# ZrrSkywalker/MonoDETR

Measured on NVIDIA H100. Metric: images/sec (1280x384, fwd+bwd), higher is better.
Workload: dtype f32 (BF16x3: error-compensated bf16 tensor-core products, fp32 accumulate)

## Files before the change

monodetr_b200/csrc/conv_gemm.cu:

```cuda
#include <cuda.h>
#include <cuda_runtime.h>
#include <stdint.h>
#include <stdlib.h>
#include <string.h>

#include "../../include/monodetr_b200.h"
#include "launch.cuh"
#include "tc_common.cuh"
#include "tma_host.cuh"

namespace {

using namespace mdb;

constexpr int BM = 128;
constexpr int BK = 32;
constexpr int kTileABytes = BM * 128;
constexpr int kChunkBytes = 32 * 128;
constexpr int kConsumerThreads = 256;
constexpr int kThreadsTC = kConsumerThreads + 32;
constexpr int kMaxTaps = 9;

struct TcParams {
    int tiles_x, tiles_y, tw, th, tb;
    int Ho, Wo;
    int out_sy, out_sx, out_oy, out_ox, out_H, out_W;
    int in_sy, in_sx;
    int ntaps, cblocks;
    int tap_dy[kMaxTaps], tap_dx[kMaxTaps], tap_w[kMaxTaps];
    int rtiles_x, rtiles_y, rtw, rth, n_img, red_per_split;
    int kb_per_slice, slice_stride;
    int total_tiles, n_tiles_n, n_tiles_m;
    int w_sy, w_sx, wg_taps, wg_kw, wg_pad;
    int Mo_rows;
    int No, ldo;
    int relu, atomic_out, round_out;
    int epi_tma, epi_load, half_x, half_y, half_b;
    const float* bias;
    const float* residual;
    const float* relu_mask;
    const float* rowscale;
    float* out;
};

template <bool MN>
__device__ __forceinline__ uint32_t raw_off(int row, int k) {
    if constexpr (MN) return (uint32_t)((row >> 5) * kChunkBytes + k * 128 + (((((row & 31) >> 2) ^ (k & 7))) << 4) + (row & 3) * 4);
    else return (uint32_t)(row * 128 + (((k >> 2) ^ (row & 7)) << 4) + (k & 3) * 4);
}

__device__ __forceinline__ float trunc_tf32(float x) { return __uint_as_float(__float_as_uint(x) & 0xFFFFE000u); }

template <int BN, int STAGES, int MODE, int PREC>
struct TcSmem {
    static constexpr bool kConvB = !(PREC == 2 && MODE == 0);
    static constexpr int kRing = STAGES * (kTileABytes + BN * 128);
    static constexpr int kStage = 2 * 64 * BN * 4;
    static constexpr int kConv = kConvB ? (PREC == 1 ? 2 : 1) * BN * 128 : 0;
    static constexpr int kFixed = kRing + kConv + 1024  + 256 ;
    static constexpr bool kTmaEpi = MODE == 0 && kFixed + kStage <= 227 * 1024;
    static constexpr int kBytes = kFixed + (kTmaEpi ? kStage : 0);
};

template <int BN, int STAGES, int MODE , bool B_MN, int PREC>
__global__ void __launch_bounds__(kThreadsTC, 1)
tc_conv_gemm_kernel(const __grid_constant__ CUtensorMap mapA, const __grid_constant__ CUtensorMap mapB,
                    const __grid_constant__ CUtensorMap mapO, const __grid_constant__ CUtensorMap mapR,
                    const __grid_constant__ TcParams p) {
    constexpr bool A_MN = (MODE == 1);
    static_assert(!(MODE == 1) || B_MN, "wgrad reads both operands MN-major");
    static_assert(BN == 64 || BN == 128, "tile width");
    constexpr bool BF_B = (PREC == 2 && MODE == 0);
    static_assert(!BF_B || !B_MN, "pre-split weights are K-major");
    constexpr bool CONVB = !BF_B;
    constexpr int kTileBBytes = BN * 128;
    constexpr int kRawBytes = kTileABytes + kTileBBytes;
    using SM = TcSmem<BN, STAGES, MODE, PREC>;
    constexpr int NACC = BN / 2;

    extern __shared__ __align__(1024) uint8_t smem[];
    uint8_t* stage_out = smem + STAGES * kRawBytes;
    uint8_t* bconv = stage_out + (SM::kTmaEpi ? SM::kStage : 0);
    uint64_t* full_bar = reinterpret_cast<uint64_t*>(bconv + SM::kConv);
    uint64_t* empty_bar = full_bar + STAGES;
    uint64_t* epi_bar = empty_bar + STAGES;

    const int warp = threadIdx.x >> 5;
    const int lane = threadIdx.x & 31;

    struct Tile { int n0, img, y0, x0, m0, red_begin, iters, tap, slice; };
    auto decode = [&](int tix) {
        Tile t;
        t.n0 = (tix % p.n_tiles_n) * BN;
        int r = tix / p.n_tiles_n;
        t.img = t.y0 = t.x0 = t.m0 = t.red_begin = t.tap = t.slice = 0;
        if constexpr (MODE == 0) {
            const int per_img = p.tiles_x * p.tiles_y;
            t.iters = p.ntaps * p.cblocks;
            if (p.kb_per_slice > 0) {
                t.slice = r / p.n_tiles_m;
                r -= t.slice * p.n_tiles_m;
                t.red_begin = t.slice * p.kb_per_slice;
                t.iters = max(0, min(t.iters, t.red_begin + p.kb_per_slice) - t.red_begin);
            }
            const int grp = r / per_img;
            t.img = grp * p.tb;
            r -= grp * per_img;
            t.y0 = (r / p.tiles_x) * p.th;
            t.x0 = (r % p.tiles_x) * p.tw;
        } else {
            t.m0 = (r % p.n_tiles_m) * BM;
// ... 34 lines not shown
                const Tile t = decode(tix);
                for (int it = 0; it < t.iters; ++it, ++git) {
                    const int s = git % STAGES;
                    const uint32_t ph = (git / STAGES) & 1;
                    mbar_wait(&empty_bar[s], ph ^ 1);
                    uint8_t* a_dst = smem + s * kRawBytes;
                    uint8_t* b_dst = a_dst + kTileABytes;
                    mbar_arrive_expect_tx(&full_bar[s], kRawBytes);
                    if constexpr (MODE == 0) {
                        const int kit = t.red_begin + it;
                        const int tap = kit / p.cblocks;
                        const int cb = kit - tap * p.cblocks;
                        tma_load_4d(a_dst, &mapA, &full_bar[s], cb * BK, t.x0 * p.in_sx + p.tap_dx[tap],
                                    t.y0 * p.in_sy + p.tap_dy[tap], t.img);
                        if constexpr (BF_B) {
                            tma_load_3d(b_dst, &mapB, &full_bar[s], cb * 64, t.n0, p.tap_w[tap]);
                        } else if constexpr (!B_MN) {
                            tma_load_3d(b_dst, &mapB, &full_bar[s], cb * BK, t.n0, p.tap_w[tap]);
                        } else {
#pragma unroll
                            for (int j = 0; j < BN / 32; ++j)
                                tma_load_3d(b_dst + j * kChunkBytes, &mapB, &full_bar[s], t.n0 + j * 32, cb * BK, p.tap_w[tap]);
                        }
                    } else {
                        int r = t.red_begin + it;
                        const int per_img = p.rtiles_x * p.rtiles_y;
                        const int ri = r / per_img;
                        r -= ri * per_img;
                        const int ry = (r / p.rtiles_x) * p.rth;
                        const int rx = (r % p.rtiles_x) * p.rtw;
#pragma unroll
                        for (int j = 0; j < BM / 32; ++j)
                            tma_load_4d(a_dst + j * kChunkBytes, &mapA, &full_bar[s], t.m0 + j * 32, rx, ry, ri);
#pragma unroll
                        for (int j = 0; j < BN / 32; ++j)
                            tma_load_4d(b_dst + j * kChunkBytes, &mapB, &full_bar[s], t.n0 + j * 32,
                                        rx * p.w_sx + (t.tap % p.wg_kw) - p.wg_pad, ry * p.w_sy + (t.tap / p.wg_kw) - p.wg_pad, ri);
                    }
                }
            }
        }
        return;
    }
    if (warp > kConsumerThreads / 32) return;

    const int wg = warp >> 2;
    const int g = lane >> 2, tig = lane & 3;
    const int r0 = wg * 64 + (warp & 3) * 16 + g;
    const int ctid = threadIdx.x;
    const bool epi_tma = SM::kTmaEpi && p.epi_tma;
    const bool leader = (ctid & 127) == 0;
    uint8_t* my_stage = stage_out + wg * (SM::kStage / 2);
    uint32_t epi_phase = 0;
    int git = 0;
    for (int tix = blockIdx.x; tix < p.total_tiles; tix += gridDim.x) {
        const Tile t = decode(tix);
        if (p.atomic_out && t.iters == 0) continue;
        const int c1 = t.x0 + wg * p.half_x, c2 = t.y0 + wg * p.half_y, c3 = t.img + wg * p.half_b, c4 = t.slice;
        if (epi_tma && p.epi_load && leader) {
            bulk_wait_read_all();
            mbar_arrive_expect_tx(&epi_bar[wg], SM::kStage / 2);
#pragma unroll
            for (int c = 0; c < BN / 32; ++c) tma_load_5d(my_stage + c * 8192, &mapR, &epi_bar[wg], t.n0 + 32 * c, c1, c2, c3, c4);
        }
        float acc[NACC];
#pragma unroll
        for (int i = 0; i < NACC; ++i) acc[i] = 0.f;
        for (int it = 0; it < t.iters; ++it, ++git) {
            const int s = git % STAGES;
            const uint32_t ph = (git / STAGES) & 1;
            mbar_wait(&full_bar[s], ph);
            const uint8_t* a_raw = smem + s * kRawBytes;
            const uint8_t* b_raw = a_raw + kTileABytes;
            if constexpr (CONVB) {
                named_bar_sync(1, kConsumerThreads);
                if constexpr (PREC == 2) {
#pragma unroll
                    for (int i = ctid; i < BN * 4; i += kConsumerThreads) {
                        const int n = i % BN, c = i / BN;
                        float x[8];
#pragma unroll
                        for (int e = 0; e < 8; ++e) x[e] = *reinterpret_cast<const float*>(b_raw + raw_off<B_MN>(n, 8 * c + e));
                        uint32_t hw[4], lw[4];
#pragma unroll
                        for (int e = 0; e < 4; ++e) {
                            const uint32_t h = pack_bf16x2(x[2 * e], x[2 * e + 1]);
                            hw[e] = h;
                            lw[e] = pack_bf16x2(x[2 * e] - __uint_as_float(h << 16), x[2 * e + 1] - __uint_as_float(h & 0xFFFF0000u));
                        }
                        uint8_t* brow = bconv + n * 128;
                        *reinterpret_cast<uint4*>(brow + ((c ^ (n & 7)) << 4)) = make_uint4(hw[0], hw[1], hw[2], hw[3]);
                        *reinterpret_cast<uint4*>(brow + (((4 + c) ^ (n & 7)) << 4)) = make_uint4(lw[0], lw[1], lw[2], lw[3]);
                    }
                } else {
#pragma unroll 4
                    for (int i = ctid; i < BN * 8; i += kConsumerThreads) {
                        const int n = i % BN, c = i / BN;
                        float4 x;
                        if constexpr (B_MN) {
                            x.x = *reinterpret_cast<const float*>(b_raw + raw_off<true>(n, 4 * c));
                            x.y = *reinterpret_cast<const float*>(b_raw + raw_off<true>(n, 4 * c + 1));
                            x.z = *reinterpret_cast<const float*>(b_raw + raw_off<true>(n, 4 * c + 2));
                            x.w = *reinterpret_cast<const float*>(b_raw + raw_off<true>(n, 4 * c + 3));
                        } else {
                            x = *reinterpret_cast<const float4*>(b_raw + raw_off<false>(n, 4 * c));
                        }
                        const float4 h = make_float4(trunc_tf32(x.x), trunc_tf32(x.y), trunc_tf32(x.z), trunc_tf32(x.w));
                        const uint32_t off = n * 128 + ((c ^ (n & 7)) << 4);
                        *reinterpret_cast<float4*>(bconv + off) = h;
                        if constexpr (PREC == 1)
                            *reinterpret_cast<float4*>(bconv + kTileBBytes + off) = make_float4(x.x - h.x, x.y - h.y, x.z - h.z, x.w - h.w);
                    }
                }
                fence_proxy_async_smem();
                named_bar_sync(1, kConsumerThreads);
            }
            const uint32_t b_addr = smem_u32(CONVB ? bconv : b_raw);
            constexpr int KS = PREC == 2 ? 2 : 4;
            uint32_t ahi[KS][4], alo[KS][4];
#pragma unroll
            for (int ks = 0; ks < KS; ++ks) {
#pragma unroll
                for (int f = 0; f < 4; ++f) {
                    const int row = r0 + (f & 1) * 8;
                    if constexpr (PREC == 2) {
                        const int k = ks * 16 + tig * 2 + (f >> 1) * 8;
                        float x0, x1;
                        if constexpr (A_MN) {
                            x0 = *reinterpret_cast<const float*>(a_raw + raw_off<true>(row, k));
                            x1 = *reinterpret_cast<const float*>(a_raw + raw_off<true>(row, k + 1));
                        } else {
                            const float2 v = *reinterpret_cast<const float2*>(a_raw + raw_off<false>(row, k));
                            x0 = v.x; x1 = v.y;
                        }
                        const uint32_t h = pack_bf16x2(x0, x1);
                        ahi[ks][f] = h;
                        alo[ks][f] = pack_bf16x2(x0 - __uint_as_float(h << 16), x1 - __uint_as_float(h & 0xFFFF0000u));
                    } else {
                        const int k = ks * 8 + tig + (f >> 1) * 4;
                        const float x = *reinterpret_cast<const float*>(a_raw + raw_off<A_MN>(row, k));
                        const float h = trunc_tf32(x);
                        ahi[ks][f] = __float_as_uint(h);
                        alo[ks][f] = __float_as_uint(x - h);
                    }
                }
            }
            wgmma_fence();
#pragma unroll
            for (int ks = 0; ks < KS; ++ks) {
                const uint64_t bhi = make_wgmma_desc_sw128(b_addr + ks * 32);
                const uint64_t blo = make_wgmma_desc_sw128(b_addr + (PREC == 2 ? 64 : kTileBBytes) + ks * 32);
                if constexpr (PREC == 2) {
                    if constexpr (BN == 128) {
                        wgmma_bf16_n128(acc, ahi[ks], bhi, 1);
                        wgmma_bf16_n128(acc, alo[ks], bhi, 1);
                        wgmma_bf16_n128(acc, ahi[ks], blo, 1);
                    } else {
                        wgmma_bf16_n64(acc, ahi[ks], bhi, 1);
                        wgmma_bf16_n64(acc, alo[ks], bhi, 1);
                        wgmma_bf16_n64(acc, ahi[ks], blo, 1);
                    }
                } else {
                    if constexpr (BN == 128) wgmma_tf32_n128(acc, ahi[ks], bhi, 1);
                    else wgmma_tf32_n64(acc, ahi[ks], bhi, 1);
                    if constexpr (PREC == 1) {
                        if constexpr (BN == 128) {
                            wgmma_tf32_n128(acc, alo[ks], bhi, 1);
                            wgmma_tf32_n128(acc, ahi[ks], blo, 1);
                        } else {
                            wgmma_tf32_n64(acc, alo[ks], bhi, 1);
                            wgmma_tf32_n64(acc, ahi[ks], blo, 1);
                        }
                    }
                }
            }
            wgmma_commit();
            wgmma_wait_all();
            wgmma_fence_operands(acc);
            __syncwarp();
            if (lane == 0) mbar_arrive(&empty_bar[s]);
        }

        if (epi_tma) {
            if (p.epi_load) {
                mbar_wait(&epi_bar[wg], epi_phase);
                epi_phase ^= 1;
            } else {
                if (leader) bulk_wait_read_all();
                named_bar_sync(2 + wg, 128);
            }
#pragma unroll
            for (int h = 0; h < 2; ++h) {
                const int row = r0 + h * 8, rr = row - 64 * wg;
                const float* gmask = nullptr;
                if (p.relu_mask && p.epi_load != 2) {
                    const int lyt = row / p.tw, lx = row - lyt * p.tw;
                    const int ib = lyt / p.th, ly = lyt - ib * p.th;
                    const int y = t.y0 + ly, x = t.x0 + lx, img = t.img + ib;
                    if ((y < p.Ho) && (x < p.Wo) && (img < p.n_img))
                        gmask = p.relu_mask + (size_t)((img * p.out_H + y * p.out_sy + p.out_oy) * p.out_W + x * p.out_sx + p.out_ox) * p.ldo;
                }
#pragma unroll
                for (int j = 0; j < BN / 8; ++j) {
                    const int n = t.n0 + j * 8 + tig * 2;
                    if (n >= p.No) continue;
                    float2* sp = reinterpret_cast<float2*>(my_stage + (j >> 2) * 8192 + raw_off<false>(rr, (j & 3) * 8 + tig * 2));
                    float v[2] = {acc[4 * j + 2 * h], acc[4 * j + 2 * h + 1]};
                    if (p.bias) { v[0] += p.bias[n]; v[1] += p.bias[n + 1]; }
                    if (p.epi_load == 1) { const float2 e = *sp; v[0] += e.x; v[1] += e.y; }
                    if (p.relu) { v[0] = fmaxf(v[0], 0.f); v[1] = fmaxf(v[1], 0.f); }
                    if (p.relu_mask) {
                        float2 m = make_float2(0.f, 0.f);
                        if (p.epi_load == 2) m = *sp;
                        else if (gmask) m = *reinterpret_cast<const float2*>(gmask + n);
                        v[0] = m.x > 0.f ? v[0] : 0.f; v[1] = m.y > 0.f ? v[1] : 0.f;
                    }
                    if (p.round_out) { v[0] = round_tf32(v[0]); v[1] = round_tf32(v[1]); }
                    *sp = make_float2(v[0], v[1]);
                }
            }
            fence_proxy_async_smem();
            named_bar_sync(2 + wg, 128);
            if (leader) {
#pragma unroll
                for (int c = 0; c < BN / 32; ++c) tma_store_5d(&mapO, my_stage + c * 8192, t.n0 + 32 * c, c1, c2, c3, c4);
                bulk_commit();
            }
            continue;
        }
#pragma unroll
        for (int h = 0; h < 2; ++h) {
            const int row = r0 + h * 8;
            bool ok;
            size_t roff;
            float rsc = 1.f;
            if constexpr (MODE == 0) {
                const int lyt = row / p.tw, lx = row - lyt * p.tw;
                const int ib = lyt / p.th, ly = lyt - ib * p.th;
                const int y = t.y0 + ly, x = t.x0 + lx, img = t.img + ib;
                ok = (y < p.Ho) && (x < p.Wo) && (img < p.n_img);
                const int oy = y * p.out_sy + p.out_oy, ox = x * p.out_sx + p.out_ox;
                roff = (size_t)((img * p.out_H + oy) * p.out_W + ox) * p.ldo + (size_t)t.slice * p.slice_stride;
            } else {
                ok = (t.m0 + row) < p.Mo_rows;
                if (ok && p.rowscale) rsc = p.rowscale[t.m0 + row];
                roff = (size_t)(t.tap * p.Mo_rows + t.m0 + row) * p.ldo;
            }
            if (!ok) continue;
            const bool vec = !(p.ldo & 1);
#pragma unroll
            for (int j = 0; j < BN / 8; ++j) {
                const int n = t.n0 + j * 8 + tig * 2;
                if (n >= p.No) continue;
                float v[2] = {acc[4 * j + 2 * h] * rsc, acc[4 * j + 2 * h + 1] * rsc};
                const bool pair = vec && n + 1 < p.No;
                if (p.bias) { v[0] += p.bias[n]; if (pair) v[1] += p.bias[n + 1]; }
                if (p.residual) {
                    if (pair) { const float2 e = *reinterpret_cast<const float2*>(p.residual + roff + n); v[0] += e.x; v[1] += e.y; }
                    else v[0] += p.residual[roff + n];
                }
                if (p.relu) { v[0] = fmaxf(v[0], 0.f); v[1] = fmaxf(v[1], 0.f); }
                if (p.relu_mask) {
                    if (pair) {
                        const float2 m = *reinterpret_cast<const float2*>(p.relu_mask + roff + n);
                        v[0] = m.x > 0.f ? v[0] : 0.f; v[1] = m.y > 0.f ? v[1] : 0.f;
                    } else {
                        v[0] = p.relu_mask[roff + n] > 0.f ? v[0] : 0.f;
                    }
                }
                if (p.round_out) { v[0] = round_tf32(v[0]); v[1] = round_tf32(v[1]); }
                float* dst = p.out + roff + n;
// ... 91 lines not shown
void pick_tile(int W, int H, int n_pix, int* tw, int* th) {
    int best_tw = n_pix, best_waste = 1 << 30;
    for (int w = n_pix; w >= 1; w >>= 1) {
        const int h = n_pix / w;
        const int tx = (W + w - 1) / w, ty = (H + h - 1) / h;
        const int waste = tx * w * ty * h - W * H;
        if (waste < best_waste) { best_waste = waste; best_tw = w; }
    }
    *tw = best_tw;
    *th = n_pix / best_tw;
}

void pick_tile3(int W, int H, int B, int n_pix, int* tw, int* th, int* tb) {
    long long best = -1;
    *tw = n_pix; *th = 1; *tb = 1;
    for (int b = 1; b <= n_pix; b <<= 1)
        for (int w = n_pix / b; w >= 1; w >>= 1) {
            const int h = n_pix / b / w;
            if (b > 1 && b >= 2 * B) continue;
            const long long cov = (long long)((W + w - 1) / w) * w * ((H + h - 1) / h) * h * ((B + b - 1) / b) * b;
            if (best < 0 || cov < best) { best = cov; *tw = w; *th = h; *tb = b; }
        }
}

bool aligned16(const void* q) { return (reinterpret_cast<uintptr_t>(q) & 15u) == 0; }

int setup_epi_px(TcParams& p, CUtensorMap* mo, CUtensorMap* mr, size_t off, int Wc, int Hc, int B, uint64_t sx, uint64_t sy,
                 uint64_t sb, int slices) {
    p.epi_tma = p.epi_load = p.half_x = p.half_y = p.half_b = 0;
    if (p.No % 4 || p.ldo % 4 || !aligned16(p.out + off) || (p.residual && !aligned16(p.residual + off)) ||
        (p.relu_mask && !aligned16(p.relu_mask + off)))
        return 0;
    uint32_t box[5] = {32, (uint32_t)p.tw, (uint32_t)p.th, (uint32_t)p.tb, 1};
    if (p.tb > 1) p.half_b = box[3] = p.tb / 2;
    else if (p.th > 1) p.half_y = box[2] = p.th / 2;
    else p.half_x = box[1] = p.tw / 2;
    if (box[1] > 256 || box[2] > 256 || box[3] > 256) return 0;
    uint64_t dims[5] = {(uint64_t)p.No, (uint64_t)Wc, (uint64_t)Hc, (uint64_t)B, (uint64_t)slices};
    uint64_t str[5] = {1, sx, sy, sb, slices > 1 ? (uint64_t)p.slice_stride : sb * B};
    int rc = make_map(mo, p.out + off, 5, dims, str, box, nullptr);
    if (rc) return rc;
    const float* opnd = p.residual ? p.residual : p.relu_mask;
    if (opnd) {
        rc = make_map(mr, opnd + off, 5, dims, str, box, nullptr);
        if (rc) return rc;
        p.epi_load = p.residual ? 1 : 2;
    }
    p.epi_tma = 1;
    return 0;
}

int launch_fwd(const CUtensorMap& ma, const CUtensorMap& mb, const CUtensorMap& mo, const CUtensorMap& mr, const TcParams& p, dim3 grid, int bn, int precision, cudaStream_t stream) {
    if (precision == 2) return bn == 64 ? launch_tc<64, 6, 0, false, 2>(ma, mb, mo, mr, p, grid, stream) : launch_tc<128, 5, 0, false, 2>(ma, mb, mo, mr, p, grid, stream);
    if (precision == 1) return bn == 64 ? launch_tc<64, 5, 0, false, 1>(ma, mb, mo, mr, p, grid, stream) : launch_tc<128, 4, 0, false, 1>(ma, mb, mo, mr, p, grid, stream);
    return bn == 64 ? launch_tc<64, 6, 0, false, 0>(ma, mb, mo, mr, p, grid, stream) : launch_tc<128, 5, 0, false, 0>(ma, mb, mo, mr, p, grid, stream);
}

struct ConvGeom {
    int B, H, W, Cin, Cout, kh, kw, stride, pad, Ho, Wo;
};

int check_geom(const ConvGeom& g, bool forward = false) {
    if (g.B <= 0 || g.H <= 0 || g.W <= 0 || g.Cin <= 0 || g.Cout <= 0) return MDB_EINVAL;
    if (g.kh != g.kw || (g.kh != 1 && g.kh != 3) || (g.stride != 1 && g.stride != 2)) return MDB_EUNSUPPORTED;
    if (g.Cin % 4 || (!forward && g.Cout % 4)) return MDB_EUNSUPPORTED;
    return 0;
}

}

extern "C" {

int mdb_set_precision(int mode) {
    if (mode < 0 || mode > 2) return MDB_EINVAL;
    g_precision = mode;
    return 0;
}
int mdb_get_precision(void) { return g_precision; }

}

namespace {

int forward_splitk_slices(int precision, int kblocks, int bn, bool plain_epilogue, int Cout, long long out_elems) {
    const int kb_per_slice = 32;
    if (precision == 0 || bn != 128 || kblocks < 256 || !plain_epilogue || Cout % 4) return 0;
    const int slices = (kblocks + kb_per_slice - 1) / kb_per_slice;
    return (out_elems * slices < (1ll << 31)) ? slices : 0;
}

int conv_forward_impl(const float* x, const void* w_packed, bool bf, const float* bias, const float* residual, float* y,
                      int B, int H, int W, int Cin, int Cout, int kh, int kw, int stride, int pad, int flags,
                      void* stream_, size_t* query_ws = nullptr ) {
    const int precision = bf ? 2 : (g_precision == 2 ? 1 : g_precision);
    ConvGeom g{B, H, W, Cin, Cout, kh, kw, stride, pad, (H + 2 * pad - kh) / stride + 1, (W + 2 * pad - kw) / stride + 1};
    int rc = check_geom(g, true);
    if (rc) return rc;
    if (!query_ws && (!x || !w_packed || !y)) return MDB_EINVAL;
    if ((unsigned long long)B * g.Ho * g.Wo * Cout >= (1ull << 31)) return MDB_EUNSUPPORTED;
    cudaStream_t stream = static_cast<cudaStream_t>(stream_);
    if (kh == 1 && stride == 1 && pad == 0) {
        W = B * H * W; H = 1; B = 1;
        g = ConvGeom{B, H, W, Cin, Cout, kh, kw, stride, pad, H, W};
    }
    TcParams p;
    memset(&p, 0, sizeof(p));
    pick_tile3(g.Wo, g.Ho, B, BM, &p.tw, &p.th, &p.tb);
// ... 106 lines not shown
            p.Ho = Hc; p.Wo = Wc;
            p.out_sy = p.out_sx = stride; p.out_oy = py; p.out_ox = px; p.out_H = H; p.out_W = W;
            p.in_sy = p.in_sx = 1;
            p.cblocks = (Cout + BK - 1) / BK;
            int nt = 0;
            for (int ky = 0; ky < kh; ++ky) {
                if ((py + pad - ky) % stride) continue;
                for (int kx = 0; kx < kw; ++kx) {
                    if ((px + pad - kx) % stride) continue;
                    p.tap_dy[nt] = (py + pad - ky) / stride;
                    p.tap_dx[nt] = (px + pad - kx) / stride;
                    p.tap_w[nt] = ky * kw + kx;
                    ++nt;
                }
            }
            p.ntaps = nt;
            p.wg_taps = 1; p.wg_kw = 1;
            p.No = Cin; p.ldo = Cin; p.relu = 0; p.atomic_out = 0; p.round_out = (precision == 0) ? ((flags >> 1) & 1) : 0;
            p.bias = nullptr; p.residual = residual; p.relu_mask = relu_mask; p.rowscale = nullptr; p.out = dx;
            CUtensorMap ma, mb;
            {
                uint64_t dims[4] = {(uint64_t)Cout, (uint64_t)g.Wo, (uint64_t)g.Ho, (uint64_t)B};
                uint64_t str[4] = {1, (uint64_t)Cout, (uint64_t)g.Wo * Cout, (uint64_t)g.Ho * g.Wo * Cout};
                uint32_t box[4] = {BK, (uint32_t)p.tw, (uint32_t)p.th, (uint32_t)p.tb};
                rc = make_map(&ma, dy, 4, dims, str, box, nullptr);
                if (rc) return rc;
            }
            const int bn = (bf && Cin <= 64) ? 64 : 128;
            if (bf) {
                const uint64_t kb = (uint64_t)p.cblocks;
                uint64_t dims[3] = {64 * kb, (uint64_t)Cin, (uint64_t)(kh * kw)};
                uint64_t str[3] = {1, 64 * kb, (uint64_t)Cin * 64 * kb};
                uint32_t box[3] = {64, (uint32_t)bn, 1};
                rc = make_map(&mb, w_packed, 3, dims, str, box, nullptr, true);
                if (rc) return rc;
            } else {
                uint64_t dims[3] = {(uint64_t)Cin, (uint64_t)Cout, (uint64_t)(kh * kw)};
                uint64_t str[3] = {1, (uint64_t)Cin, (uint64_t)Cout * Cin};
                uint32_t box[3] = {32, 32, 1};
                rc = make_map(&mb, w_packed, 3, dims, str, box, nullptr);
                if (rc) return rc;
            }
            dim3 grid((Cin + bn - 1) / bn, n_groups * p.tiles_x * p.tiles_y, 1);
            if (nt == 0) {
                p.ntaps = 0;
            }
            CUtensorMap mo, mr;
            memset(&mo, 0, sizeof(mo));
            memset(&mr, 0, sizeof(mr));
            rc = setup_epi_px(p, &mo, &mr, (size_t)(py * W + px) * Cin, Wc, Hc, B, (uint64_t)stride * Cin,
                              (uint64_t)stride * W * Cin, (uint64_t)H * W * Cin, 1);
            if (rc) return rc;
            if (bf) rc = launch_fwd(ma, mb, mo, mr, p, grid, bn, 2, stream);
            else rc = (precision == 1) ? launch_tc<128, 4, 0, true, 1>(ma, mb, mo, mr, p, grid, stream)
                                       : launch_tc<128, 5, 0, true, 0>(ma, mb, mo, mr, p, grid, stream);
            if (rc) return rc;
        }
    return 0;
}

}

extern "C" {

int mdb_conv2d_forward_f32(const float* x, const float* w_packed, const float* bias, const float* residual, float* y,
                           int B, int H, int W, int Cin, int Cout, int kh, int kw, int stride, int pad, int flags,
                           void* stream) {
    return conv_forward_impl(x, w_packed, false, bias, residual, y, B, H, W, Cin, Cout, kh, kw, stride, pad, flags, stream);
}
int mdb_conv2d_forward_bf16x3(const float* x, const void* w_split, const float* bias, const float* residual, float* y,
                              int B, int H, int W, int Cin, int Cout, int kh, int kw, int stride, int pad, int flags,
                              void* stream) {
    return conv_forward_impl(x, w_split, true, bias, residual, y, B, H, W, Cin, Cout, kh, kw, stride, pad, flags, stream);
}
long long mdb_conv2d_forward_workspace_bytes(int B, int H, int W, int Cin, int Cout, int kh, int kw, int stride, int pad,
                                             int flags, int has_residual, int split_weights) {
    size_t bytes = 0;
    const float* res = has_residual ? reinterpret_cast<const float*>(16) : nullptr;
    const int rc = conv_forward_impl(nullptr, nullptr, split_weights != 0, nullptr, res, nullptr, B, H, W, Cin, Cout, kh, kw, stride,
                                     pad, flags, nullptr, &bytes);
    return rc ? (long long)rc : (long long)bytes;
}
int mdb_set_workspace(void* buf, unsigned long long bytes) {
    DeviceState& d = g_dev[current_device()];
    d.ws = static_cast<float*>(buf);
    d.ws_bytes = buf ? (size_t)bytes : 0;
    return 0;
}
int mdb_conv2d_dgrad_f32(const float* dy, const float* w_packed, const float* residual, const float* relu_mask,
                         float* dx, int B, int H, int W, int Cin, int Cout, int kh, int kw, int stride, int pad,
                         int flags, void* stream) {
    return conv_dgrad_impl(dy, w_packed, false, residual, relu_mask, dx, B, H, W, Cin, Cout, kh, kw, stride, pad, flags, stream);
}
int mdb_conv2d_dgrad_bf16x3(const float* dy, const void* w_split_t, const float* residual, const float* relu_mask,
                            float* dx, int B, int H, int W, int Cin, int Cout, int kh, int kw, int stride, int pad,
                            int flags, void* stream) {
    return conv_dgrad_impl(dy, w_split_t, true, residual, relu_mask, dx, B, H, W, Cin, Cout, kh, kw, stride, pad, flags, stream);
}

int mdb_conv2d_wgrad_f32(const float* dy, const float* x, const float* rowscale, float* dw_packed, int B, int H, int W,
                         int Cin, int Cout, int kh, int kw, int stride, int pad, int accumulate, void* stream_) {
    return mdb_conv2d_wgrad_bias_f32(dy, x, rowscale, dw_packed, nullptr, B, H, W, Cin, Cout, kh, kw, stride, pad, accumulate, stream_);
}

int mdb_conv2d_wgrad_bias_f32(const float* dy, const float* x, const float* rowscale, float* dw_packed, float* db, int B, int H,
                              int W, int Cin, int Cout, int kh, int kw, int stride, int pad, int accumulate, void* stream_) {
    ConvGeom g{B, H, W, Cin, Cout, kh, kw, stride, pad, (H + 2 * pad - kh) / stride + 1, (W + 2 * pad - kw) / stride + 1};
// ... 69 lines not shown
```

monodetr_b200/csrc/tc_common.cuh:

```cuda
#pragma once
#include <cuda.h>
#include <cuda_runtime.h>
#include <stdint.h>

namespace mdb {

__device__ __forceinline__ uint32_t smem_u32(const void* p) {
    return static_cast<uint32_t>(__cvta_generic_to_shared(p));
}

__device__ __forceinline__ bool elect_one() {
    uint32_t pred = 0;
    asm volatile(
        "{\n\t.reg .b32 rx;\n\t.reg .pred px;\n\t"
        "elect.sync rx|px, 0xffffffff;\n\t"
        "selp.b32 %0, 1, 0, px;\n\t}"
        : "=r"(pred));
    return pred != 0;
}

__device__ __forceinline__ void mbar_init(uint64_t* bar, uint32_t count) {
    asm volatile("mbarrier.init.shared::cta.b64 [%0], %1;" ::"r"(smem_u32(bar)), "r"(count) : "memory");
}
__device__ __forceinline__ void fence_mbar_init() {
// ... 32 lines not shown
        }
    }
}

__device__ __forceinline__ void fence_proxy_async_smem() { asm volatile("fence.proxy.async.shared::cta;" ::: "memory"); }
__device__ __forceinline__ void named_bar_sync(int id, int count) { asm volatile("bar.sync %0, %1;" ::"r"(id), "r"(count) : "memory"); }

__device__ __forceinline__ void tma_prefetch_desc(const CUtensorMap* m) {
    asm volatile("prefetch.tensormap [%0];" ::"l"(reinterpret_cast<uint64_t>(m)) : "memory");
}
__device__ __forceinline__ void tma_load_2d(void* dst, const CUtensorMap* m, uint64_t* bar, int c0, int c1) {
    asm volatile(
        "cp.async.bulk.tensor.2d.shared::cluster.global.mbarrier::complete_tx::bytes [%0], [%1, {%3, %4}], [%2];" ::"r"(
            smem_u32(dst)),
        "l"(reinterpret_cast<uint64_t>(m)), "r"(smem_u32(bar)), "r"(c0), "r"(c1)
        : "memory");
}
__device__ __forceinline__ void tma_load_3d(void* dst, const CUtensorMap* m, uint64_t* bar, int c0, int c1, int c2) {
    asm volatile(
        "cp.async.bulk.tensor.3d.shared::cluster.global.mbarrier::complete_tx::bytes [%0], [%1, {%3, %4, %5}], [%2];" ::"r"(
            smem_u32(dst)),
        "l"(reinterpret_cast<uint64_t>(m)), "r"(smem_u32(bar)), "r"(c0), "r"(c1), "r"(c2)
        : "memory");
}
__device__ __forceinline__ void tma_load_4d(void* dst, const CUtensorMap* m, uint64_t* bar, int c0, int c1, int c2,
                                            int c3) {
    asm volatile(
        "cp.async.bulk.tensor.4d.shared::cluster.global.mbarrier::complete_tx::bytes [%0], [%1, {%3, %4, %5, %6}], "
        "[%2];" ::"r"(smem_u32(dst)),
        "l"(reinterpret_cast<uint64_t>(m)), "r"(smem_u32(bar)), "r"(c0), "r"(c1), "r"(c2), "r"(c3)
        : "memory");
}
__device__ __forceinline__ void tma_load_5d(void* dst, const CUtensorMap* m, uint64_t* bar, int c0, int c1, int c2,
                                            int c3, int c4) {
    asm volatile(
        "cp.async.bulk.tensor.5d.shared::cluster.global.mbarrier::complete_tx::bytes [%0], [%1, {%3, %4, %5, %6, %7}], "
        "[%2];" ::"r"(smem_u32(dst)),
        "l"(reinterpret_cast<uint64_t>(m)), "r"(smem_u32(bar)), "r"(c0), "r"(c1), "r"(c2), "r"(c3), "r"(c4)
        : "memory");
}
__device__ __forceinline__ void tma_store_5d(const CUtensorMap* m, const void* src, int c0, int c1, int c2, int c3, int c4) {
    asm volatile("cp.async.bulk.tensor.5d.global.shared::cta.bulk_group [%0, {%2, %3, %4, %5, %6}], [%1];"
                 ::"l"(reinterpret_cast<uint64_t>(m)), "r"(smem_u32(src)), "r"(c0), "r"(c1), "r"(c2), "r"(c3), "r"(c4)
                 : "memory");
}
__device__ __forceinline__ void bulk_commit() { asm volatile("cp.async.bulk.commit_group;" ::: "memory"); }
__device__ __forceinline__ void bulk_wait_read_all() { asm volatile("cp.async.bulk.wait_group.read 0;" ::: "memory"); }
__device__ __forceinline__ void bulk_wait_all() { asm volatile("cp.async.bulk.wait_group 0;" ::: "memory"); }

__device__ __forceinline__ void wgmma_fence() { asm volatile("wgmma.fence.sync.aligned;" ::: "memory"); }
__device__ __forceinline__ void wgmma_commit() { asm volatile("wgmma.commit_group.sync.aligned;" ::: "memory"); }
__device__ __forceinline__ void wgmma_wait_all() { asm volatile("wgmma.wait_group.sync.aligned 0;" ::: "memory"); }
template <int N>
__device__ __forceinline__ void wgmma_fence_operands(float (&d)[N]) {
#pragma unroll
    for (int i = 0; i < N; ++i) asm volatile("" : "+f"(d[i])::"memory");
}
__device__ __forceinline__ void wgmma_bf16_n64(float (&d)[32], const uint32_t (&a)[4], uint64_t bdesc, int scale_d) {
    asm volatile(
        "{\n\t.reg .pred p;\n\t"
        "setp.ne.b32 p, %37, 0;\n\t"
        "wgmma.mma_async.sync.aligned.m64n64k16.f32.bf16.bf16 "
        "{%0, %1, %2, %3, %4, %5, %6, %7, %8, %9, %10, %11, %12, %13, %14, %15, "
        "%16, %17, %18, %19, %20, %21, %22, %23, %24, %25, %26, %27, %28, %29, %30, %31"
        "}, {%32, %33, %34, %35}, %36, p, 1, 1, 0;\n\t}"
        : "+f"(d[0]), "+f"(d[1]), "+f"(d[2]), "+f"(d[3]), "+f"(d[4]), "+f"(d[5]), "+f"(d[6]), "+f"(d[7]), "+f"(d[8]), "+f"(d[9]), "+f"(d[10]), "+f"(d[11]), "+f"(d[12]), "+f"(d[13]), "+f"(d[14]), "+f"(d[15]), "+f"(d[16]), "+f"(d[17]), "+f"(d[18]), "+f"(d[19]), "+f"(d[20]), "+f"(d[21]), "+f"(d[22]), "+f"(d[23]), "+f"(d[24]), "+f"(d[25]), "+f"(d[26]), "+f"(d[27]), "+f"(d[28]), "+f"(d[29]), "+f"(d[30]), "+f"(d[31])
        : "r"(a[0]), "r"(a[1]), "r"(a[2]), "r"(a[3]), "l"(bdesc), "r"(scale_d));
}
__device__ __forceinline__ void wgmma_bf16_n128(float (&d)[64], const uint32_t (&a)[4], uint64_t bdesc, int scale_d) {
    asm volatile(
        "{\n\t.reg .pred p;\n\t"
        "setp.ne.b32 p, %69, 0;\n\t"
        "wgmma.mma_async.sync.aligned.m64n128k16.f32.bf16.bf16 "
        "{%0, %1, %2, %3, %4, %5, %6, %7, %8, %9, %10, %11, %12, %13, %14, %15, "
        "%16, %17, %18, %19, %20, %21, %22, %23, %24, %25, %26, %27, %28, %29, %30, %31, "
        "%32, %33, %34, %35, %36, %37, %38, %39, %40, %41, %42, %43, %44, %45, %46, %47, "
        "%48, %49, %50, %51, %52, %53, %54, %55, %56, %57, %58, %59, %60, %61, %62, %63"
        "}, {%64, %65, %66, %67}, %68, p, 1, 1, 0;\n\t}"
        : "+f"(d[0]), "+f"(d[1]), "+f"(d[2]), "+f"(d[3]), "+f"(d[4]), "+f"(d[5]), "+f"(d[6]), "+f"(d[7]), "+f"(d[8]), "+f"(d[9]), "+f"(d[10]), "+f"(d[11]), "+f"(d[12]), "+f"(d[13]), "+f"(d[14]), "+f"(d[15]), "+f"(d[16]), "+f"(d[17]), "+f"(d[18]), "+f"(d[19]), "+f"(d[20]), "+f"(d[21]), "+f"(d[22]), "+f"(d[23]), "+f"(d[24]), "+f"(d[25]), "+f"(d[26]), "+f"(d[27]), "+f"(d[28]), "+f"(d[29]), "+f"(d[30]), "+f"(d[31]), "+f"(d[32]), "+f"(d[33]), "+f"(d[34]), "+f"(d[35]), "+f"(d[36]), "+f"(d[37]), "+f"(d[38]), "+f"(d[39]), "+f"(d[40]), "+f"(d[41]), "+f"(d[42]), "+f"(d[43]), "+f"(d[44]), "+f"(d[45]), "+f"(d[46]), "+f"(d[47]), "+f"(d[48]), "+f"(d[49]), "+f"(d[50]), "+f"(d[51]), "+f"(d[52]), "+f"(d[53]), "+f"(d[54]), "+f"(d[55]), "+f"(d[56]), "+f"(d[57]), "+f"(d[58]), "+f"(d[59]), "+f"(d[60]), "+f"(d[61]), "+f"(d[62]), "+f"(d[63])
        : "r"(a[0]), "r"(a[1]), "r"(a[2]), "r"(a[3]), "l"(bdesc), "r"(scale_d));
}
__device__ __forceinline__ void wgmma_tf32_n32(float (&d)[16], const uint32_t (&a)[4], uint64_t bdesc, int scale_d) {
    asm volatile(
        "{\n\t.reg .pred p;\n\t"
        "setp.ne.b32 p, %21, 0;\n\t"
        "wgmma.mma_async.sync.aligned.m64n32k8.f32.tf32.tf32 "
        "{%0, %1, %2, %3, %4, %5, %6, %7, %8, %9, %10, %11, %12, %13, %14, %15"
        "}, {%16, %17, %18, %19}, %20, p, 1, 1;\n\t}"
        : "+f"(d[0]), "+f"(d[1]), "+f"(d[2]), "+f"(d[3]), "+f"(d[4]), "+f"(d[5]), "+f"(d[6]), "+f"(d[7]), "+f"(d[8]), "+f"(d[9]), "+f"(d[10]), "+f"(d[11]), "+f"(d[12]), "+f"(d[13]), "+f"(d[14]), "+f"(d[15])
        : "r"(a[0]), "r"(a[1]), "r"(a[2]), "r"(a[3]), "l"(bdesc), "r"(scale_d));
}

__device__ __forceinline__ void wgmma_tf32_n64(float (&d)[32], const uint32_t (&a)[4], uint64_t bdesc, int scale_d) {
    asm volatile(
        "{\n\t.reg .pred p;\n\t"
        "setp.ne.b32 p, %37, 0;\n\t"
        "wgmma.mma_async.sync.aligned.m64n64k8.f32.tf32.tf32 "
        "{%0, %1, %2, %3, %4, %5, %6, %7, %8, %9, %10, %11, %12, %13, %14, %15, "
        "%16, %17, %18, %19, %20, %21, %22, %23, %24, %25, %26, %27, %28, %29, %30, %31"
        "}, {%32, %33, %34, %35}, %36, p, 1, 1;\n\t}"
        : "+f"(d[0]), "+f"(d[1]), "+f"(d[2]), "+f"(d[3]), "+f"(d[4]), "+f"(d[5]), "+f"(d[6]), "+f"(d[7]), "+f"(d[8]), "+f"(d[9]), "+f"(d[10]), "+f"(d[11]), "+f"(d[12]), "+f"(d[13]), "+f"(d[14]), "+f"(d[15]), "+f"(d[16]), "+f"(d[17]), "+f"(d[18]), "+f"(d[19]), "+f"(d[20]), "+f"(d[21]), "+f"(d[22]), "+f"(d[23]), "+f"(d[24]), "+f"(d[25]), "+f"(d[26]), "+f"(d[27]), "+f"(d[28]), "+f"(d[29]), "+f"(d[30]), "+f"(d[31])
        : "r"(a[0]), "r"(a[1]), "r"(a[2]), "r"(a[3]), "l"(bdesc), "r"(scale_d));
}
__device__ __forceinline__ void wgmma_tf32_n128(float (&d)[64], const uint32_t (&a)[4], uint64_t bdesc, int scale_d) {
    asm volatile(
        "{\n\t.reg .pred p;\n\t"
        "setp.ne.b32 p, %69, 0;\n\t"
        "wgmma.mma_async.sync.aligned.m64n128k8.f32.tf32.tf32 "
        "{%0, %1, %2, %3, %4, %5, %6, %7, %8, %9, %10, %11, %12, %13, %14, %15, "
// ... 35 lines not shown
```

Before: 157.6.

## Software-pipeline wgmma issue with next k-block fragment prep and double-buffered B conversion

The consumer loop now issues the wgmma group for k-block i and keeps it in flight with wait_group<1> while it converts the next k-block's A fragments and B tile into a second conversion buffer. Previously every iteration waited for all wgmmas before any further work, so conversion and tensor-core work ran back to back. The empty-barrier release for a stage is deferred by one iteration. To pay for the doubled conversion buffer, the stage count of the precision-1 BN=128 variants drops from 4 to 3. The epilogue also hoists the bias add and batches the relu-mask global loads.

```diff
diff --git a/monodetr_b200/csrc/conv_gemm.cu b/monodetr_b200/csrc/conv_gemm.cu
--- a/monodetr_b200/csrc/conv_gemm.cu
+++ b/monodetr_b200/csrc/conv_gemm.cu
@@ -56,7 +56,8 @@
     static constexpr bool kConvB = !(PREC == 2 && MODE == 0);
     static constexpr int kRing = STAGES * (kTileABytes + BN * 128);
     static constexpr int kStage = 2 * 64 * BN * 4;
-    static constexpr int kConv = kConvB ? (PREC == 1 ? 2 : 1) * BN * 128 : 0;
+    static constexpr int kConvBuf = kConvB ? (PREC == 1 ? 2 : 1) * BN * 128 : 0;
+    static constexpr int kConv = 2 * kConvBuf;
     static constexpr int kFixed = kRing + kConv + 1024  + 256 ;
     static constexpr bool kTmaEpi = MODE == 0 && kFixed + kStage <= 227 * 1024;
     static constexpr int kBytes = kFixed + (kTmaEpi ? kStage : 0);
@@ -197,6 +198,118 @@
     const bool leader = (ctid & 127) == 0;
     uint8_t* my_stage = stage_out + wg * (SM::kStage / 2);
     uint32_t epi_phase = 0;
+    constexpr int KS = PREC == 2 ? 2 : 4;
+    using Frag = uint32_t[KS][4];
+    auto load_kblock = [&](int gi, int buf, Frag& hi, Frag& lo) {
+        const int s = gi % STAGES;
+        mbar_wait(&full_bar[s], (gi / STAGES) & 1);
+        const uint8_t* a_raw = smem + s * kRawBytes;
+        if constexpr (CONVB) {
+            const uint8_t* b_raw = a_raw + kTileABytes;
+            uint8_t* bc = bconv + buf * SM::kConvBuf;
+            named_bar_sync(1, kConsumerThreads);
+            if constexpr (PREC == 2) {
+#pragma unroll
+                for (int i = ctid; i < BN * 4; i += kConsumerThreads) {
+                    const int n = i % BN, c = i / BN;
+                    float x[8];
+#pragma unroll
+                    for (int e = 0; e < 8; ++e) x[e] = *reinterpret_cast<const float*>(b_raw + raw_off<B_MN>(n, 8 * c + e));
+                    uint32_t hw[4], lw[4];
+#pragma unroll
+                    for (int e = 0; e < 4; ++e) {
+                        const uint32_t h = pack_bf16x2(x[2 * e], x[2 * e + 1]);
+                        hw[e] = h;
+                        lw[e] = pack_bf16x2(x[2 * e] - __uint_as_float(h << 16), x[2 * e + 1] - __uint_as_float(h & 0xFFFF0000u));
+                    }
+                    uint8_t* brow = bc + n * 128;
+                    *reinterpret_cast<uint4*>(brow + ((c ^ (n & 7)) << 4)) = make_uint4(hw[0], hw[1], hw[2], hw[3]);
+                    *reinterpret_cast<uint4*>(brow + (((4 + c) ^ (n & 7)) << 4)) = make_uint4(lw[0], lw[1], lw[2], lw[3]);
+                }
+            } else {
+#pragma unroll 4
+                for (int i = ctid; i < BN * 8; i += kConsumerThreads) {
+                    const int n = i % BN, c = i / BN;
+                    float4 x;
+                    if constexpr (B_MN) {
+                        x.x = *reinterpret_cast<const float*>(b_raw + raw_off<true>(n, 4 * c));
+                        x.y = *reinterpret_cast<const float*>(b_raw + raw_off<true>(n, 4 * c + 1));
+                        x.z = *reinterpret_cast<const float*>(b_raw + raw_off<true>(n, 4 * c + 2));
+                        x.w = *reinterpret_cast<const float*>(b_raw + raw_off<true>(n, 4 * c + 3));
+                    } else {
+                        x = *reinterpret_cast<const float4*>(b_raw + raw_off<false>(n, 4 * c));
+                    }
+                    const float4 h = make_float4(trunc_tf32(x.x), trunc_tf32(x.y), trunc_tf32(x.z), trunc_tf32(x.w));
+                    const uint32_t off = n * 128 + ((c ^ (n & 7)) << 4);
+                    *reinterpret_cast<float4*>(bc + off) = h;
+                    if constexpr (PREC == 1)
+                        *reinterpret_cast<float4*>(bc + kTileBBytes + off) = make_float4(x.x - h.x, x.y - h.y, x.z - h.z, x.w - h.w);
+                }
+            }
+            fence_proxy_async_smem();
+            named_bar_sync(1, kConsumerThreads);
+        }
+#pragma unroll
+        for (int ks = 0; ks < KS; ++ks) {
+#pragma unroll
+            for (int f = 0; f < 4; ++f) {
+                const int row = r0 + (f & 1) * 8;
+                if constexpr (PREC == 2) {
+                    const int k = ks * 16 + tig * 2 + (f >> 1) * 8;
+                    float x0, x1;
+                    if constexpr (A_MN) {
+                        x0 = *reinterpret_cast<const float*>(a_raw + raw_off<true>(row, k));
+                        x1 = *reinterpret_cast<const float*>(a_raw + raw_off<true>(row, k + 1));
+                    } else {
+                        const float2 v = *reinterpret_cast<const float2*>(a_raw + raw_off<false>(row, k));
+                        x0 = v.x; x1 = v.y;
+                    }
+                    const uint32_t h = pack_bf16x2(x0, x1);
+                    hi[ks][f] = h;
+                    lo[ks][f] = pack_bf16x2(x0 - __uint_as_float(h << 16), x1 - __uint_as_float(h & 0xFFFF0000u));
+                } else {
+                    const int k = ks * 8 + tig + (f >> 1) * 4;
+                    const float x = *reinterpret_cast<const float*>(a_raw + raw_off<A_MN>(row, k));
+                    const float h = trunc_tf32(x);
+                    hi[ks][f] = __float_as_uint(h);
+                    lo[ks][f] = __float_as_uint(x - h);
+                }
+            }
+        }
+    };
+    auto issue_kblock = [&](int gi, int buf, const Frag& hi, const Frag& lo, float (&acc)[NACC]) {
+        const uint32_t b_addr = smem_u32(CONVB ? bconv + buf * SM::kConvBuf : smem + (gi % STAGES) * kRawBytes + kTileABytes);
+        wgmma_fence();
+#pragma unroll
+        for (int ks = 0; ks < KS; ++ks) {
+            const uint64_t bhi = make_wgmma_desc_sw128(b_addr + ks * 32);
+            const uint64_t blo = make_wgmma_desc_sw128(b_addr + (PREC == 2 ? 64 : kTileBBytes) + ks * 32);
+            if constexpr (PREC == 2) {
+                if constexpr (BN == 128) {
+                    wgmma_bf16_n128(acc, hi[ks], bhi, 1);
+                    wgmma_bf16_n128(acc, lo[ks], bhi, 1);
+                    wgmma_bf16_n128(acc, hi[ks], blo, 1);
+                } else {
+                    wgmma_bf16_n64(acc, hi[ks], bhi, 1);
+                    wgmma_bf16_n64(acc, lo[ks], bhi, 1);
+                    wgmma_bf16_n64(acc, hi[ks], blo, 1);
+                }
+            } else {
+                if constexpr (BN == 128) wgmma_tf32_n128(acc, hi[ks], bhi, 1);
+                else wgmma_tf32_n64(acc, hi[ks], bhi, 1);
+                if constexpr (PREC == 1) {
+                    if constexpr (BN == 128) {
+                        wgmma_tf32_n128(acc, lo[ks], bhi, 1);
+                        wgmma_tf32_n128(acc, hi[ks], blo, 1);
+                    } else {
+                        wgmma_tf32_n64(acc, lo[ks], bhi, 1);
+                        wgmma_tf32_n64(acc, hi[ks], blo, 1);
+                    }
+                }
+            }
+        }
+        wgmma_commit();
+    };
     int git = 0;
     for (int tix = blockIdx.x; tix < p.total_tiles; tix += gridDim.x) {
         const Tile t = decode(tix);
@@ -211,122 +324,45 @@
         float acc[NACC];
 #pragma unroll
         for (int i = 0; i < NACC; ++i) acc[i] = 0.f;
-        for (int it = 0; it < t.iters; ++it, ++git) {
-            const int s = git % STAGES;
-            const uint32_t ph = (git / STAGES) & 1;
-            mbar_wait(&full_bar[s], ph);
-            const uint8_t* a_raw = smem + s * kRawBytes;
-            const uint8_t* b_raw = a_raw + kTileABytes;
-            if constexpr (CONVB) {
-                named_bar_sync(1, kConsumerThreads);
-                if constexpr (PREC == 2) {
-#pragma unroll
-                    for (int i = ctid; i < BN * 4; i += kConsumerThreads) {
-                        const int n = i % BN, c = i / BN;
-                        float x[8];
-#pragma unroll
-                        for (int e = 0; e < 8; ++e) x[e] = *reinterpret_cast<const float*>(b_raw + raw_off<B_MN>(n, 8 * c + e));
-                        uint32_t hw[4], lw[4];
-#pragma unroll
-                        for (int e = 0; e < 4; ++e) {
-                            const uint32_t h = pack_bf16x2(x[2 * e], x[2 * e + 1]);
-                            hw[e] = h;
-                            lw[e] = pack_bf16x2(x[2 * e] - __uint_as_float(h << 16), x[2 * e + 1] - __uint_as_float(h & 0xFFFF0000u));
-                        }
-                        uint8_t* brow = bconv + n * 128;
-                        *reinterpret_cast<uint4*>(brow + ((c ^ (n & 7)) << 4)) = make_uint4(hw[0], hw[1], hw[2], hw[3]);
-                        *reinterpret_cast<uint4*>(brow + (((4 + c) ^ (n & 7)) << 4)) = make_uint4(lw[0], lw[1], lw[2], lw[3]);
-                    }
-                } else {
-#pragma unroll 4
-                    for (int i = ctid; i < BN * 8; i += kConsumerThreads) {
-                        const int n = i % BN, c = i / BN;
-                        float4 x;
-                        if constexpr (B_MN) {
-                            x.x = *reinterpret_cast<const float*>(b_raw + raw_off<true>(n, 4 * c));
-                            x.y = *reinterpret_cast<const float*>(b_raw + raw_off<true>(n, 4 * c + 1));
-                            x.z = *reinterpret_cast<const float*>(b_raw + raw_off<true>(n, 4 * c + 2));
-                            x.w = *reinterpret_cast<const float*>(b_raw + raw_off<true>(n, 4 * c + 3));
-                        } else {
-                            x = *reinterpret_cast<const float4*>(b_raw + raw_off<false>(n, 4 * c));
-                        }
-                        const float4 h = make_float4(trunc_tf32(x.x), trunc_tf32(x.y), trunc_tf32(x.z), trunc_tf32(x.w));
-                        const uint32_t off = n * 128 + ((c ^ (n & 7)) << 4);
-                        *reinterpret_cast<float4*>(bconv + off) = h;
-                        if constexpr (PREC == 1)
-                            *reinterpret_cast<float4*>(bconv + kTileBBytes + off) = make_float4(x.x - h.x, x.y - h.y, x.z - h.z, x.w - h.w);
-                    }
-                }
-                fence_proxy_async_smem();
-                named_bar_sync(1, kConsumerThreads);
-            }
-            const uint32_t b_addr = smem_u32(CONVB ? bconv : b_raw);
-            constexpr int KS = PREC == 2 ? 2 : 4;
-            uint32_t ahi[KS][4], alo[KS][4];
-#pragma unroll
-            for (int ks = 0; ks < KS; ++ks) {
-#pragma unroll
-                for (int f = 0; f < 4; ++f) {
-                    const int row = r0 + (f & 1) * 8;
-                    if constexpr (PREC == 2) {
-                        const int k = ks * 16 + tig * 2 + (f >> 1) * 8;
-                        float x0, x1;
-                        if constexpr (A_MN) {
-                            x0 = *reinterpret_cast<const float*>(a_raw + raw_off<true>(row, k));
-                            x1 = *reinterpret_cast<const float*>(a_raw + raw_off<true>(row, k + 1));
-                        } else {
-                            const float2 v = *reinterpret_cast<const float2*>(a_raw + raw_off<false>(row, k));
-                            x0 = v.x; x1 = v.y;
-                        }
-                        const uint32_t h = pack_bf16x2(x0, x1);
-                        ahi[ks][f] = h;
-                        alo[ks][f] = pack_bf16x2(x0 - __uint_as_float(h << 16), x1 - __uint_as_float(h & 0xFFFF0000u));
-                    } else {
-                        const int k = ks * 8 + tig + (f >> 1) * 4;
-                        const float x = *reinterpret_cast<const float*>(a_raw + raw_off<A_MN>(row, k));
-                        const float h = trunc_tf32(x);
-                        ahi[ks][f] = __float_as_uint(h);
-                        alo[ks][f] = __float_as_uint(x - h);
-                    }
-                }
-            }
-            wgmma_fence();
-#pragma unroll
-            for (int ks = 0; ks < KS; ++ks) {
-                const uint64_t bhi = make_wgmma_desc_sw128(b_addr + ks * 32);
-                const uint64_t blo = make_wgmma_desc_sw128(b_addr + (PREC == 2 ? 64 : kTileBBytes) + ks * 32);
-                if constexpr (PREC == 2) {
-                    if constexpr (BN == 128) {
-                        wgmma_bf16_n128(acc, ahi[ks], bhi, 1);
-                        wgmma_bf16_n128(acc, alo[ks], bhi, 1);
-                        wgmma_bf16_n128(acc, ahi[ks], blo, 1);
-                    } else {
-                        wgmma_bf16_n64(acc, ahi[ks], bhi, 1);
-                        wgmma_bf16_n64(acc, alo[ks], bhi, 1);
-                        wgmma_bf16_n64(acc, ahi[ks], blo, 1);
-                    }
-                } else {
-                    if constexpr (BN == 128) wgmma_tf32_n128(acc, ahi[ks], bhi, 1);
-                    else wgmma_tf32_n64(acc, ahi[ks], bhi, 1);
-                    if constexpr (PREC == 1) {
-                        if constexpr (BN == 128) {
-                            wgmma_tf32_n128(acc, alo[ks], bhi, 1);
-                            wgmma_tf32_n128(acc, ahi[ks], blo, 1);
-                        } else {
-                            wgmma_tf32_n64(acc, alo[ks], bhi, 1);
-                            wgmma_tf32_n64(acc, ahi[ks], blo, 1);
-                        }
-                    }
-                }
-            }
-            wgmma_commit();
-            wgmma_wait_all();
+        if (t.iters > 0) {
+            Frag ahi0, alo0, ahi1, alo1;
+            auto step = [&](int it, const Frag& chi, const Frag& clo, Frag& nhi, Frag& nlo) {
+                issue_kblock(git + it, it & 1, chi, clo, acc);
+                wgmma_wait<1>();
+                wgmma_fence_operands(nhi);
+                wgmma_fence_operands(nlo);
+                if (it > 0) {
+                    __syncwarp();
+                    if (lane == 0) mbar_arrive(&empty_bar[(git + it - 1) % STAGES]);
+                }
+                if (it + 1 < t.iters) load_kblock(git + it + 1, (it + 1) & 1, nhi, nlo);
+            };
+            load_kblock(git, 0, ahi0, alo0);
+            for (int it = 0; it < t.iters; it += 2) {
+                step(it, ahi0, alo0, ahi1, alo1);
+                if (it + 1 < t.iters) step(it + 1, ahi1, alo1, ahi0, alo0);
+            }
+            wgmma_wait<0>();
             wgmma_fence_operands(acc);
+            wgmma_fence_operands(ahi0);
+            wgmma_fence_operands(alo0);
+            wgmma_fence_operands(ahi1);
+            wgmma_fence_operands(alo1);
             __syncwarp();
-            if (lane == 0) mbar_arrive(&empty_bar[s]);
+            if (lane == 0) mbar_arrive(&empty_bar[(git + t.iters - 1) % STAGES]);
+            git += t.iters;
         }
 
         if (epi_tma) {
+            if (p.bias) {
+#pragma unroll
+                for (int j = 0; j < BN / 8; ++j) {
+                    const int n = t.n0 + j * 8 + tig * 2;
+                    if (n >= p.No) continue;
+                    const float b0 = p.bias[n], b1 = p.bias[n + 1];
+                    acc[4 * j] += b0; acc[4 * j + 1] += b1; acc[4 * j + 2] += b0; acc[4 * j + 3] += b1;
+                }
+            }
             if (p.epi_load) {
                 mbar_wait(&epi_bar[wg], epi_phase);
                 epi_phase ^= 1;
@@ -334,6 +370,7 @@
                 if (leader) bulk_wait_read_all();
                 named_bar_sync(2 + wg, 128);
             }
+            constexpr int kMB = 8;
 #pragma unroll
             for (int h = 0; h < 2; ++h) {
                 const int row = r0 + h * 8, rr = row - 64 * wg;
@@ -346,22 +383,28 @@
                         gmask = p.relu_mask + (size_t)((img * p.out_H + y * p.out_sy + p.out_oy) * p.out_W + x * p.out_sx + p.out_ox) * p.ldo;
                 }
 #pragma unroll
-                for (int j = 0; j < BN / 8; ++j) {
-                    const int n = t.n0 + j * 8 + tig * 2;
-                    if (n >= p.No) continue;
-                    float2* sp = reinterpret_cast<float2*>(my_stage + (j >> 2) * 8192 + raw_off<false>(rr, (j & 3) * 8 + tig * 2));
-                    float v[2] = {acc[4 * j + 2 * h], acc[4 * j + 2 * h + 1]};
-                    if (p.bias) { v[0] += p.bias[n]; v[1] += p.bias[n + 1]; }
-                    if (p.epi_load == 1) { const float2 e = *sp; v[0] += e.x; v[1] += e.y; }
-                    if (p.relu) { v[0] = fmaxf(v[0], 0.f); v[1] = fmaxf(v[1], 0.f); }
-                    if (p.relu_mask) {
-                        float2 m = make_float2(0.f, 0.f);
-                        if (p.epi_load == 2) m = *sp;
-                        else if (gmask) m = *reinterpret_cast<const float2*>(gmask + n);
-                        v[0] = m.x > 0.f ? v[0] : 0.f; v[1] = m.y > 0.f ? v[1] : 0.f;
+                for (int j0 = 0; j0 < BN / 8; j0 += kMB) {
+                    float2 mv[kMB];
+#pragma unroll
+                    for (int u = 0; u < kMB; ++u) {
+                        const int n = t.n0 + (j0 + u) * 8 + tig * 2;
+                        mv[u] = (gmask && n < p.No) ? *reinterpret_cast<const float2*>(gmask + n) : make_float2(0.f, 0.f);
                     }
-                    if (p.round_out) { v[0] = round_tf32(v[0]); v[1] = round_tf32(v[1]); }
-                    *sp = make_float2(v[0], v[1]);
+#pragma unroll
+                    for (int u = 0; u < kMB; ++u) {
+                        const int j = j0 + u, n = t.n0 + j * 8 + tig * 2;
+                        if (n >= p.No) continue;
+                        float2* sp = reinterpret_cast<float2*>(my_stage + (j >> 2) * 8192 + raw_off<false>(rr, (j & 3) * 8 + tig * 2));
+                        float v[2] = {acc[4 * j + 2 * h], acc[4 * j + 2 * h + 1]};
+                        if (p.epi_load == 1) { const float2 e = *sp; v[0] += e.x; v[1] += e.y; }
+                        if (p.relu) { v[0] = fmaxf(v[0], 0.f); v[1] = fmaxf(v[1], 0.f); }
+                        if (p.relu_mask) {
+                            const float2 m = p.epi_load == 2 ? *sp : mv[u];
+                            v[0] = m.x > 0.f ? v[0] : 0.f; v[1] = m.y > 0.f ? v[1] : 0.f;
+                        }
+                        if (p.round_out) { v[0] = round_tf32(v[0]); v[1] = round_tf32(v[1]); }
+                        *sp = make_float2(v[0], v[1]);
+                    }
                 }
             }
             fence_proxy_async_smem();
@@ -559,7 +602,7 @@
 
 int launch_fwd(const CUtensorMap& ma, const CUtensorMap& mb, const CUtensorMap& mo, const CUtensorMap& mr, const TcParams& p, dim3 grid, int bn, int precision, cudaStream_t stream) {
     if (precision == 2) return bn == 64 ? launch_tc<64, 6, 0, false, 2>(ma, mb, mo, mr, p, grid, stream) : launch_tc<128, 5, 0, false, 2>(ma, mb, mo, mr, p, grid, stream);
-    if (precision == 1) return bn == 64 ? launch_tc<64, 5, 0, false, 1>(ma, mb, mo, mr, p, grid, stream) : launch_tc<128, 4, 0, false, 1>(ma, mb, mo, mr, p, grid, stream);
+    if (precision == 1) return bn == 64 ? launch_tc<64, 5, 0, false, 1>(ma, mb, mo, mr, p, grid, stream) : launch_tc<128, 3, 0, false, 1>(ma, mb, mo, mr, p, grid, stream);
     return bn == 64 ? launch_tc<64, 6, 0, false, 0>(ma, mb, mo, mr, p, grid, stream) : launch_tc<128, 5, 0, false, 0>(ma, mb, mo, mr, p, grid, stream);
 }
 
@@ -772,7 +815,7 @@
                               (uint64_t)stride * W * Cin, (uint64_t)H * W * Cin, 1);
             if (rc) return rc;
             if (bf) rc = launch_fwd(ma, mb, mo, mr, p, grid, bn, 2, stream);
-            else rc = (precision == 1) ? launch_tc<128, 4, 0, true, 1>(ma, mb, mo, mr, p, grid, stream)
+            else rc = (precision == 1) ? launch_tc<128, 3, 0, true, 1>(ma, mb, mo, mr, p, grid, stream)
                                        : launch_tc<128, 5, 0, true, 0>(ma, mb, mo, mr, p, grid, stream);
             if (rc) return rc;
         }
diff --git a/monodetr_b200/csrc/tc_common.cuh b/monodetr_b200/csrc/tc_common.cuh
--- a/monodetr_b200/csrc/tc_common.cuh
+++ b/monodetr_b200/csrc/tc_common.cuh
@@ -108,9 +108,18 @@
 __device__ __forceinline__ void wgmma_commit() { asm volatile("wgmma.commit_group.sync.aligned;" ::: "memory"); }
 __device__ __forceinline__ void wgmma_wait_all() { asm volatile("wgmma.wait_group.sync.aligned 0;" ::: "memory"); }
 template <int N>
+__device__ __forceinline__ void wgmma_wait() { asm volatile("wgmma.wait_group.sync.aligned %0;" ::"n"(N) : "memory"); }
+template <int N>
 __device__ __forceinline__ void wgmma_fence_operands(float (&d)[N]) {
 #pragma unroll
     for (int i = 0; i < N; ++i) asm volatile("" : "+f"(d[i])::"memory");
+}
+template <int M, int N>
+__device__ __forceinline__ void wgmma_fence_operands(uint32_t (&a)[M][N]) {
+#pragma unroll
+    for (int i = 0; i < M; ++i)
+#pragma unroll
+        for (int j = 0; j < N; ++j) asm volatile("" : "+r"(a[i][j])::"memory");
 }
 __device__ __forceinline__ void wgmma_bf16_n64(float (&d)[32], const uint32_t (&a)[4], uint64_t bdesc, int scale_d) {
     asm volatile(
```

Result: faster. 168.8, median of 6 (+7.1%).
